# rust-cv/cv

Measured on NVIDIA H100. Metric: vSLAM frames/s (AKAZE+match+RANSAC, 1080p ~5k kp) at 1/2/4/8 H100, higher is better.
Workload: dtype f32+f64

## Files before the change

cv_b200/csrc/akaze.cu:

```cuda
#include <math.h>
#include <stdarg.h>
#include <stdio.h>
#include <stdlib.h>
#include <string.h>
#include <algorithm>
#include <atomic>
#include <vector>
#include "../../include/cvb200_stages.h"
#include "akaze_kernels.cuh"
#include "common.cuh"

using namespace akz;

namespace {

struct EvoHost {
    int w = 0, h = 0;
    uint32_t octave = 0, sublevel = 0;
    double esigma = 0, etime = 0;
    uint32_t sigma = 0;
    float quat = 0;
    float norm = 0, middle = 0;
    std::vector<double> tau;
    size_t off = 0;
// ... 104 lines not shown
    bool use_tma = false;
    int tma_mask = 3;
    SupScratch sup{};
    bool suppress_seq = false;
    bool suppress_par_only = false;
    unsigned *sup_fallback = nullptr;
    unsigned char *tile_evo = nullptr;
    MaskLayout mask_layout{};
    unsigned *extrema_mask = nullptr;
    bool deriv_v3 = true;
    OrientTables *ot = nullptr;
    DescTables *dt = nullptr;
    cvb_keypoint *kp_out = nullptr;
    unsigned char *desc_out = nullptr;
    unsigned *n_out = nullptr;
    unsigned cap_out = 0;
    std::vector<void *> allocs;
    std::vector<void *> kp_allocs;
    bool has_run = false;
    cudaStream_t aux = nullptr;
    cudaEvent_t ev_fork[8] = {}, ev_join = nullptr;
    struct GraphEntry { const void *img; void *kp, *desc, *n; unsigned B, cap; cudaGraphExec_t exec; };
    std::vector<GraphEntry> graphs;
    uint64_t launches_per_graph = 0;
    bool use_graph = true;
    bool use_aux = true;
    uint64_t ticket = 0;
    unsigned ss_batch = 0;
    DescTables *dt_side = nullptr;
    int dt_side_pattern = 0, dt_side_nch = 0;
    cvb_keypoint *st_kp = nullptr, *st_kp_out = nullptr;
    unsigned char *st_ok = nullptr, *st_desc = nullptr, *st_desc_out = nullptr;
    unsigned *st_off = nullptr, *st_n = nullptr, *st_need = nullptr;
    size_t st_kp_n = 0, st_kp_out_n = 0, st_ok_n = 0, st_desc_n = 0, st_desc_out_n = 0, st_off_n = 0, st_n_n = 0, st_need_n = 0;
};

void akaze_workspace_free(AkazeWorkspace *ws) {
    if (!ws) return;
    for (auto &g : ws->graphs) cudaGraphExecDestroy(g.exec);
    if (ws->aux) cudaStreamDestroy(ws->aux);
    for (cudaEvent_t e : ws->ev_fork) if (e) cudaEventDestroy(e);
    if (ws->ev_join) cudaEventDestroy(ws->ev_join);
    for (void *p : ws->allocs) cudaFree(p);
    for (void *p : ws->kp_allocs) cudaFree(p);
    for (void *p : {(void *)ws->st_kp, (void *)ws->st_kp_out, (void *)ws->st_ok, (void *)ws->st_desc, (void *)ws->st_desc_out,
                    (void *)ws->st_off, (void *)ws->st_n, (void *)ws->st_need})
        if (p) cudaFree(p);
    delete ws;
}

namespace {

#ifndef CVB_TMA_DEFAULT
#define CVB_TMA_DEFAULT 1
#endif
typedef CUresult (*EncodeTiledFn)(CUtensorMap *, CUtensorMapDataType, cuuint32_t, void *, const cuuint64_t *, const cuuint64_t *,
                                  const cuuint32_t *, const cuuint32_t *, CUtensorMapInterleave, CUtensorMapSwizzle, CUtensorMapL2promotion,
                                  CUtensorMapFloatOOBfill);
EncodeTiledFn encode_tiled_fn() {
    static EncodeTiledFn fn = nullptr;
    static bool tried = false;
    if (!tried) {
        tried = true;
        void *p = nullptr;
        cudaDriverEntryPointQueryResult qr;
        if (cudaGetDriverEntryPoint("cuTensorMapEncodeTiled", &p, cudaEnableDefault, &qr) == cudaSuccess && qr == cudaDriverEntryPointSuccess)
            fn = (EncodeTiledFn)p;
    }
    return fn;
}
bool make_tmap(CUtensorMap *out, const float *base, int w, int h, unsigned B, size_t bstride, int boxw, int boxh) {
    EncodeTiledFn fn = encode_tiled_fn();
    memset(out, 0, sizeof(*out));
    if (!fn || ((uintptr_t)base & 15) || (w & 3) || (bstride & 3) || boxw > 256 || boxh > 256 || w < 1 || h < 1) return false;
    const cuuint64_t dims[3] = {(cuuint64_t)w, (cuuint64_t)h, (cuuint64_t)std::max(B, 1u)};
    const cuuint64_t strides[2] = {(cuuint64_t)w * 4, (cuuint64_t)(B > 1 ? bstride : (size_t)w * h) * 4};
    const cuuint32_t box[3] = {(cuuint32_t)boxw, (cuuint32_t)boxh, 1};
    const cuuint32_t es[3] = {1, 1, 1};
    return fn(out, CU_TENSOR_MAP_DATA_TYPE_FLOAT32, 3, (void *)base, dims, strides, box, es, CU_TENSOR_MAP_INTERLEAVE_NONE,
              CU_TENSOR_MAP_SWIZZLE_NONE, CU_TENSOR_MAP_L2_PROMOTION_NONE, CU_TENSOR_MAP_FLOAT_OOB_FILL_NONE) == CUDA_SUCCESS;
}


int fed_fuse_steps() {
    static int v = 0;
    if (!v) { const char *env = getenv("CVB_FED_FUSE"); v = env ? std::min(std::max(atoi(env), 1), FED_SMAX) : FED_FUSE_DEFAULT; }
    return v;
}

template <typename T>
int dalloc_into(cvb_ctx *ctx, std::vector<void *> &list, T **p, size_t n) {
    void *q = nullptr;
    cudaError_t e = cudaMalloc(&q, std::max<size_t>(n, 1) * sizeof(T));
    if (e != cudaSuccess) return cvb_set_error(ctx, CVB_ENOMEM, "cudaMalloc(%zu bytes): %s", n * sizeof(T), cudaGetErrorString(e));
    list.push_back(q);
    *p = (T *)q;
    return 0;
}

template <typename T>
int dalloc(cvb_ctx *ctx, AkazeWorkspace *ws, T **p, size_t n) { return dalloc_into(ctx, ws->allocs, p, n); }

int alloc_keypoint_buffers(cvb_ctx *ctx, AkazeWorkspace *ws) {
    const size_t B = ws->batch;
    int rc = 0;
#define DK(p, n) do { rc = dalloc_into(ctx, ws->kp_allocs, &ws->p, (n)); if (rc) return rc; } while (0)
    DK(cand, B * ws->capc);
    DK(sup.state, B * ws->capc); DK(sup.alive, B * ws->capc); DK(sup.rdy, B * ws->capc);
    DK(sup.key, B * ws->capc); DK(sup.rank, B * ws->capc); DK(sup.next, B * ws->capc);
    DK(cache, B * ws->capk); DK(refined, B * ws->capk); DK(sorted, B * ws->capk); DK(rank, B * ws->capk);
    DK(keep, B * ws->capk); DK(valid, B * ws->capk); DK(ok, B * ws->capk); DK(desc_tmp, B * ws->capk * 64);
#undef DK
    return 0;
}

int grow_keypoint_capacity(cvb_ctx *ctx, AkazeWorkspace *ws, size_t need_c, size_t need_k) {
    CVB_CUDA(ctx, cvb_wait(ctx, ctx->stream));
    for (auto &g : ws->graphs) cudaGraphExecDestroy(g.exec);
    ws->graphs.clear();
    AkazeWorkspace *nw = new AkazeWorkspace();
    nw->batch = ws->batch;
    nw->capc = need_c > ws->capc ? (unsigned)std::min<size_t>(need_c + need_c / 8, 0xffffffffu) : ws->capc;
    nw->capk = need_k > ws->capk ? (unsigned)std::min<size_t>(need_k + need_k / 8, 0xffffffffu) : ws->capk;
    const int rc = alloc_keypoint_buffers(ctx, nw);
    if (rc) {
        for (void *p : nw->kp_allocs) cudaFree(p);
        delete nw;
        return rc;
    }
    for (void *p : ws->kp_allocs) cudaFree(p);
    ws->kp_allocs = std::move(nw->kp_allocs);
    ws->capc = nw->capc; ws->capk = nw->capk;
    ws->cand = nw->cand;
    ws->sup.state = nw->sup.state; ws->sup.alive = nw->sup.alive; ws->sup.rdy = nw->sup.rdy;
    ws->sup.key = nw->sup.key; ws->sup.rank = nw->sup.rank; ws->sup.next = nw->sup.next;
    ws->cache = nw->cache; ws->refined = nw->refined; ws->sorted = nw->sorted; ws->rank = nw->rank;
    ws->keep = nw->keep; ws->valid = nw->valid; ws->ok = nw->ok; ws->desc_tmp = nw->desc_tmp;
    delete nw;
    return 0;
}

bool same_cfg(const cvb_akaze_cfg &a, const cvb_akaze_cfg &b) { return memcmp(&a, &b, sizeof(a)) == 0; }

int plan_evolutions(cvb_ctx *ctx, AkazeWorkspace *ws) {
    const cvb_akaze_cfg &c = ws->cfg;
    ws->evo.clear();
    for (uint32_t octave = 0; octave < c.max_octave_evolution; octave++) {
        double rfactor = 1.0 / (double)(1ull << octave);
        uint32_t lh = (uint32_t)((double)ws->h * rfactor), lw = (uint32_t)((double)ws->w * rfactor);
        uint32_t smallest = std::min(lw, lh);
        if (smallest < 40) continue;
        uint32_t sub = smallest < 80 ? 1 : c.num_sublevels;
        for (uint32_t s = 0; s < sub; s++) {
            EvoHost e;
            e.octave = octave; e.sublevel = s;
            e.esigma = c.base_scale_offset * pow(2.0, (double)s / (double)c.num_sublevels + (double)octave);
            e.etime = 0.5 * (e.esigma * e.esigma);
            ws->evo.push_back(e);
        }
    }
    if (ws->evo.empty()) return 0;
    if (ws->evo.size() > (size_t)MAX_EVO) return cvb_set_error(ctx, CVB_EUNSUPPORTED, "more than %d evolutions", MAX_EVO);
    int lw = (int)ws->w, lh = (int)ws->h;
    size_t off = 0;
    int rowbase = 0, tilebase = 0;
    for (size_t i = 0; i < ws->evo.size(); i++) {
        EvoHost &e = ws->evo[i];
        e.new_octave = i > 0 && e.octave > ws->evo[i - 1].octave;
        if (e.new_octave) { lw /= 2; lh /= 2; }
        e.w = lw; e.h = lh; e.off = off;
        off += (size_t)lw * lh;
        off = (off + 63) & ~(size_t)63;
// ... 333 lines not shown
            dim3 g((unsigned)(t1 - t0), 1, B);
            CVB_PROF(ctx, "k_detector_response", 16.0 * px * B);
            k_detector_response<<<g, NT, sizeof(float) * det_smem_floats(smax), ds>>>(ws->Lsm, ws->Lt, ws->Lx, ws->Ly, ws->Ldet, PF, ws->table,
                                                                                      ws->tile_evo, t0, ws->mask_layout, thr, ws->extrema_mask,
                                                                                      ws->rowcount);
            CVB_LAUNCH_CHECK(ctx);
        } else if (ws->deriv_v3) {
            const size_t region = (((size_t)pitch3(smax) * (SH3 + 2 * smax)) + 31) & ~(size_t)31;
            dim3 g((unsigned)(t1 - t0), 1, B);
            { CVB_PROF(ctx, "k_deriv1", 12.0 * px * B);
            k_deriv1_v3<<<g, NT, sizeof(float) * region + 128, ds>>>(ws->Lsm, ws->Lt, ws->Lx, ws->Ly, PF, ws->table, ws->tile_evo, t0,
                                                               ws->use_tma && (ws->tma_mask & 4) ? ws->tmaps : nullptr);
            CVB_LAUNCH_CHECK(ctx); }
            { CVB_PROF(ctx, "k_deriv2_det", 12.0 * px * B);
            k_deriv2_v3<<<g, NT, sizeof(float) * 2 * region + 128, ds>>>(ws->Lx, ws->Ly, ws->Ldet, PF, ws->table, ws->tile_evo, t0,
                                                                   ws->use_tma && (ws->tma_mask & 8) ? ws->tmaps + MAX_EVO : nullptr, ws->use_tma && (ws->tma_mask & 8) ? ws->tmaps + 2 * MAX_EVO : nullptr);
            CVB_LAUNCH_CHECK(ctx); }
        } else {
            cudaStream_t keep = ctx->stream;
            ctx->stream = ds;
            int rc2 = 0;
            for (int e = e0; e < e1 && !rc2; e++) {
                const EvoHost &ev = ws->evo[e];
                rc2 = launch_deriv1(ctx, ev, (e == 0 ? ws->Lt : ws->Lsm) + ev.off, ws->Lx + ev.off, ws->Ly + ev.off, PF, B);
                if (!rc2) rc2 = launch_deriv2(ctx, ev, ws->Lx + ev.off, ws->Ly + ev.off, ws->Ldet + ev.off, PF, B);
            }
            ctx->stream = keep;
            if (rc2) return rc2;
        }
        return 0;
    };
    int octave_first = 0;
    int rc = launch_separable(ctx, images, P0, ws->Lt + ws->evo[0].off, PF, W, H, B, ws->g0, ws->g0);
    if (rc) return rc;
    CVB_CUDA(ctx, cudaMemsetAsync(ws->gmax, 0, sizeof(unsigned long long) * B, st));
    CVB_CUDA(ctx, cudaMemsetAsync(ws->hist, 0, sizeof(unsigned) * B * nbins, st));
    CVB_CUDA(ctx, cudaMemsetAsync(ws->npoints, 0, sizeof(unsigned) * B, st));
    CVB_CUDA(ctx, cudaMemsetAsync(ws->rowcount, 0, sizeof(unsigned) * (size_t)B * R, st));
    rc = launch_separable(ctx, images, P0, ws->tmpA, P0, W, H, B, ws->g1, ws->g1);
    if (rc) return rc;
    { CVB_PROF(ctx, "k_contrast_grad", 4.0 * W * H * B);
    k_scharr_pm_v3<1><<<dim3(cdiv((unsigned)W, SW3), cdiv((unsigned)H, SH3), B), NT, 0, st>>>(ws->tmpA, nullptr, ws->g2, ws->gmax, W, H, P0, P0, nullptr, 0);
    CVB_LAUNCH_CHECK(ctx); }
    {
        unsigned blocks = std::min<unsigned>(cdiv((unsigned)P0, NT), (unsigned)ctx->num_sms * 8);
        { CVB_PROF(ctx, "k_contrast_hist", 4.0 * W * H * B);
        k_contrast_hist<<<dim3(blocks, 1, B), NT, sizeof(unsigned) * nbins, st>>>(ws->g2, ws->gmax, ws->hist, ws->npoints, (int)P0, P0, nbins);
        CVB_LAUNCH_CHECK(ctx); }
        { CVB_PROF(ctx, "k_contrast_final", 0);
        k_contrast_final<<<B, 32, 0, st>>>(ws->gmax, ws->hist, ws->npoints, nbins, ws->cfg.contrast_percentile, ws->evo_octave, E, ws->kc, ws->inv_k);
        CVB_LAUNCH_CHECK(ctx); }
    }
    for (int i = 1; i < E; i++) {
        const EvoHost &e = ws->evo[i];
        const EvoHost &pe = ws->evo[i - 1];
        const float *src = ws->Lt + pe.off;
        size_t src_bs = PF;
        if (e.new_octave) {
            if ((rc = issue_detector_response(octave_first, i))) return rc;
            octave_first = i;
            dim3 blk(32, 8), grd(cdiv((unsigned)e.w, 32), cdiv((unsigned)e.h, 8), B);
            { CVB_PROF(ctx, "k_half_size", 4.0 * ((double)pe.w * pe.h + (double)e.w * e.h) * B);
            k_half_size<<<grd, blk, 0, st>>>(src, ws->tmpC, pe.w, pe.h, src_bs, P0);
            CVB_LAUNCH_CHECK(ctx); }
            src = ws->tmpC; src_bs = P0;
        }
        if (ws->fuse_blur_scharr && ws->g1.ks == 5) {
            CVB_PROF(ctx, "k_blur_scharr", 16.0 * e.w * e.h * B);
            CUtensorMap tm;
            const int use_tma = ws->use_tma && (ws->tma_mask & 2) && make_tmap(&tm, src, e.w, e.h, B, src_bs, pitch3(3), SH3 + 6) ? 1 : 0;
            if (!use_tma) memset(&tm, 0, sizeof(tm));
            k_blur_scharr_pm<<<dim3(cdiv((unsigned)e.w, SW3), cdiv((unsigned)e.h, SH3), B), NT, 0, st>>>(
                src, ws->Lsm + e.off, ws->Lflow + e.off, e.w, e.h, src_bs, PF, PF, ws->g1, ws->inv_k + i, MAX_EVO, tm, use_tma);
            CVB_LAUNCH_CHECK(ctx);
        } else {
            rc = launch_separable(ctx, src, src_bs, ws->Lsm + e.off, PF, e.w, e.h, B, ws->g1, ws->g1);
            if (rc) return rc;
            { CVB_PROF(ctx, "k_scharr_pm", 8.0 * e.w * e.h * B);
            k_scharr_pm_v3<0><<<dim3(cdiv((unsigned)e.w, SW3), cdiv((unsigned)e.h, SH3), B), NT, 0, st>>>(ws->Lsm + e.off, ws->Lflow + e.off, nullptr, nullptr, e.w, e.h, PF, PF,
                                                                 ws->inv_k + i, MAX_EVO);
            CVB_LAUNCH_CHECK(ctx); }
        }
        const int n = (int)e.tau.size();
        const int fed_fuse = fed_fuse_steps();
        const int nl = (n + fed_fuse - 1) / fed_fuse;
        if (nl == 0) {
            CVB_CUDA(ctx, cudaMemcpy2DAsync(ws->Lt + e.off, PF * sizeof(float), src, src_bs * sizeof(float),
                                            (size_t)e.w * e.h * sizeof(float), B, cudaMemcpyDeviceToDevice, st));
        }
        const float *cur = src; size_t cur_bs = src_bs;
        int done = 0;
        for (int l = 0; l < nl; l++) {
            FedSteps fs;
            fs.n = (n - done + (nl - l) - 1) / (nl - l);
            for (int t = 0; t < fs.n; t++) fs.tau[t] = (float)e.tau[(size_t)(done + t)];
            done += fs.n;
            float *dst; size_t dst_bs;
            if (l == nl - 1) { dst = ws->Lt + e.off; dst_bs = PF; }
            else if (((nl - 1 - l) & 1) == 1) { dst = ws->tmpA; dst_bs = P0; }
            else { dst = ws->tmpB; dst_bs = P0; }
            { CVB_PROF(ctx, "k_fed", 12.0 * fs.n * e.w * e.h * B);
            const int hx = (fs.n + 3) & ~3;
            dim3 grd(cdiv((unsigned)e.w, (unsigned)(F3_W - 2 * hx)), cdiv((unsigned)e.h, (unsigned)(F3_H - 2 * fs.n)), B);
            k_fed3<<<grd, F3_H * 16, 0, st>>>(cur, ws->Lflow + e.off, dst, e.w, e.h, cur_bs, PF, dst_bs, fs);
            CVB_LAUNCH_CHECK(ctx); }
            cur = dst; cur_bs = dst_bs;
        }
    }
    if ((rc = issue_detector_response(octave_first, E))) return rc;
    if (forked) {
        CVB_CUDA(ctx, cudaEventRecord(ws->ev_join, ws->aux));
        CVB_CUDA(ctx, cudaStreamWaitEvent(st, ws->ev_join, 0));
    }
    return 0;
}

int stage_detect(cvb_ctx *ctx, unsigned B) {
    AkazeWorkspace *ws = ctx->akaze;
    cudaStream_t st = ctx->stream;
    const size_t PF = ws->plane_floats;
    const bool fused_det = ws->deriv_v3 && ws->fuse_det;
    const int R = ws->table.total_rows;
    const float thr = (float)ws->cfg.detector_threshold;
    {
        if (!fused_det) { CVB_PROF(ctx, "k_extrema_mask", 4.0 * ws->plane_floats * B);
        k_extrema_mask<<<dim3((unsigned)ws->table.total_tiles, 1, B), NT, 0, st>>>(ws->Ldet, PF, ws->table, ws->tile_evo, ws->mask_layout, thr,
                                                                                    ws->extrema_mask, ws->rowcount);
        CVB_LAUNCH_CHECK(ctx); }
        { CVB_PROF(ctx, "k_scan_rows", 0);
        k_scan_rows<<<B, 1024, 0, st>>>(ws->rowcount, ws->rowoff, ws->ncand, R);
        CVB_LAUNCH_CHECK(ctx); }
        { CVB_PROF(ctx, "k_extrema_emit", 0);
        k_extrema_emit<<<dim3(cdiv((unsigned)R * 32u, NT), 1, B), NT, 0, st>>>(ws->Ldet, PF, ws->table, ws->mask_layout, ws->extrema_mask, ws->rowcount,
                                                                                 ws->rowoff, ws->cand, ws->capc, ws->overflow);
        CVB_LAUNCH_CHECK(ctx); }
    }
    { CVB_PROF(ctx, "k_suppress", 0);
    if (ws->suppress_seq)
        k_suppress_seq<<<B, 1024, 0, st>>>(ws->cand, ws->ncand, ws->capc, ws->table, ws->cache, ws->ncache, ws->nneed, ws->capk,
                                           ws->overflow);
    else {
        k_suppress_smem<<<B, 1024, SUP_SMEM, st>>>(ws->cand, ws->ncand, ws->rowoff, ws->capc, ws->table, ws->sup, ws->cache,
                                                   ws->ncache, ws->nneed, ws->capk, ws->overflow, ws->sup_fallback);
        CVB_LAUNCH_CHECK(ctx);
        k_suppress_par<<<B, 1024, 0, st>>>(ws->cand, ws->ncand, ws->rowoff, ws->capc, ws->table, ws->sup, ws->cache, ws->ncache,
                                           ws->nneed, ws->capk, ws->overflow, ws->suppress_par_only ? nullptr : ws->sup_fallback);
    }
    CVB_LAUNCH_CHECK(ctx); }
    const unsigned kp_blocks = (unsigned)ctx->num_sms * 2;
    const unsigned ichunks = std::min<unsigned>(cdiv(ws->capk, NT), 64u);
    CVB_CUDA(ctx, cudaMemsetAsync(ws->keep, 1, (size_t)B * ws->capk, st));
    { CVB_PROF(ctx, "k_filter_upper", 0);
    k_filter_upper<<<dim3(ichunks, 16, B), NT, 0, st>>>(ws->cache, ws->ncache, ws->capk, ws->keep);
    CVB_LAUNCH_CHECK(ctx); }
    { CVB_PROF(ctx, "k_refine_orient", 0);
    k_refine_orient<<<dim3(kp_blocks, B), NT, 0, st>>>(ws->cache, ws->ncache, ws->capk, ws->keep, ws->table, ws->Ldet, ws->Lx, ws->Ly, PF,
                                                       ws->ot, ws->refined, ws->valid);
    CVB_LAUNCH_CHECK(ctx); }
    return 0;
}

int stage_sort_describe(cvb_ctx *ctx, unsigned B, cvb_keypoint *kp_out, unsigned char *desc_out, unsigned cap_out, unsigned *n_out) {
    AkazeWorkspace *ws = ctx->akaze;
    cudaStream_t st = ctx->stream;
    const size_t PF = ws->plane_floats;
    const unsigned ichunks = std::min<unsigned>(cdiv(ws->capk, NT), 64u);
    CVB_CUDA(ctx, cudaMemsetAsync(ws->rank, 0, sizeof(unsigned) * (size_t)B * ws->capk, st));
    CVB_CUDA(ctx, cudaMemsetAsync(ws->nvalid, 0, sizeof(unsigned) * B, st));
    { CVB_PROF(ctx, "k_rank_sort", 0);
    k_rank_count<<<dim3(ichunks, 16, B), NT, 0, st>>>(ws->refined, ws->valid, ws->ncache, ws->capk, ws->rank);
    CVB_LAUNCH_CHECK(ctx);
    k_rank_scatter<<<dim3(ichunks, B), NT, 0, st>>>(ws->refined, ws->valid, ws->ncache, ws->capk, ws->rank,
                                                    (long long)ws->cfg.maximum_features, ws->sorted, ws->nvalid);
    CVB_LAUNCH_CHECK(ctx);
    k_clamp_count<<<cdiv(B, 32), 32, 0, st>>>(ws->nvalid, (long long)ws->cfg.maximum_features, ws->nsorted, (int)B);
    CVB_LAUNCH_CHECK(ctx); }
    { CVB_PROF(ctx, "k_descriptors", 0);
    k_descriptors<<<dim3((unsigned)ctx->num_sms * 8, B), DESC_WARPS * 32, 0, st>>>(ws->sorted, ws->nsorted, nullptr, ws->capk, ws->table, ws->Lt,
                                                     ws->Lx, ws->Ly, PF, ws->dt, (int)ws->cfg.descriptor_channels,
                                                     (int)ws->cfg.descriptor_pattern_size, ws->desc_tmp, ws->ok, ws->overflow);
    CVB_LAUNCH_CHECK(ctx); }
    { CVB_PROF(ctx, "k_compact_final", 0);
    k_compact_final<<<B, 1024, 0, st>>>(ws->sorted, ws->desc_tmp, ws->ok, ws->nsorted, ws->capk, kp_out, desc_out, cap_out, n_out,
                                        ws->overflow);
    CVB_LAUNCH_CHECK(ctx); }
    return 0;
}
// ... 486 lines not shown
```

cv_b200/csrc/akaze_kernels.cuh:

```cuda
#pragma once
#include <cuda.h>
#include <cuda/barrier>
#include <cuda_runtime.h>
#include <stdint.h>
#include "device_libm.cuh"
#include "../../include/cvb200.h"

namespace akz {

constexpr int TW = 32;
constexpr int TH = 32;
constexpr int NT = 256;
constexpr int MAXK = 33;
constexpr int MAX_EVO = 32;
constexpr int MAX_TAU = 64;
constexpr int FED_SMAX = 8, FED_FUSE_DEFAULT = 8;

struct Taps { int ks; float k[MAXK]; };

struct EvoDev {
    int w, h;
    unsigned long long off;
    int octave;
    float size;
    int rowbase;
    int tilebase;
    int sigma;
    float norm, middle;
    float quat;
    int pad;
};
struct EvoTable { int n; int total_rows; int total_tiles; int pad; EvoDev e[MAX_EVO]; };

struct Cand { int x, y, e; float v; };

__device__ __forceinline__ int clampi(int v, int lo, int hi) { return v < lo ? lo : (v > hi ? hi : v); }

__device__ __forceinline__ float lane_dot(const float *w, int stride, const float *k, int ks) {
    float l0 = 0.f, l1 = 0.f, l2 = 0.f, l3 = 0.f;
    int j = 0;
    for (; j + 4 <= ks; j += 4) {
        l0 = w[(j + 0) * stride] * k[j + 0] + l0;
        l1 = w[(j + 1) * stride] * k[j + 1] + l1;
        l2 = w[(j + 2) * stride] * k[j + 2] + l2;
        l3 = w[(j + 3) * stride] * k[j + 3] + l3;
    }
    if (j < ks) l0 = w[j * stride] * k[j] + l0;
    if (j + 1 < ks) l1 = w[(j + 1) * stride] * k[j + 1] + l1;
    if (j + 2 < ks) l2 = w[(j + 2) * stride] * k[j + 2] + l2;
    return (l0 + l2) + (l1 + l3);
}

template <int JA, int JB>
__device__ __forceinline__ float dot2(float a, float ka, float b, float kb) {
    return (a * ka + b * kb) + 0.f;
}
template <int JA, int JB, int JC>
__device__ __forceinline__ float dot3(float a, float ka, float b, float kb, float c, float kc) {
    const float pa = a * ka, pb = b * kb, pc = c * kc;
    float r;
    if (JA == JB) r = (JC == JA) ? pc + (pb + pa) : (pb + pa) + pc;
    else if (JA == JC) r = (pc + pa) + pb;
    else if (JB == JC) r = (pc + pb) + pa;
    else if ((JA ^ JB) == 2) r = (pa + pb) + pc;
    else if ((JA ^ JC) == 2) r = (pa + pc) + pb;
    else r = (pb + pc) + pa;
    return r + 0.f;
}
template <int SM>
__device__ __forceinline__ float scharr_main(float first, float last) {
    return (last - first) + 0.f;
}
template <int SM>
__device__ __forceinline__ float scharr_off(float first, float mid, float last, float norm, float middle) {
    return dot3<0, SM & 3, (2 * SM) & 3>(first, norm, mid, middle, last, norm);
}

__global__ void __launch_bounds__(NT) k_separable(const float *__restrict__ in, float *__restrict__ out, int w, int h,
                                                  size_t in_bstride, size_t out_bstride, Taps hk, Taps vk) {
    extern __shared__ float sm[];
    const int rx = hk.ks / 2, ry = vk.ks / 2;
    const int sw = TW + 2 * rx, sh = TH + 2 * ry;
    float *s_in = sm;
    float *s_h = sm + sh * sw;
    const float *src = in + (size_t)blockIdx.z * in_bstride;
    float *dst = out + (size_t)blockIdx.z * out_bstride;
    const int x0 = blockIdx.x * TW, y0 = blockIdx.y * TH;
    for (int i = threadIdx.x; i < sw * sh; i += NT) {
        int ly = i / sw, lx = i - ly * sw;
        int gx = clampi(x0 + lx - rx, 0, w - 1), gy = clampi(y0 + ly - ry, 0, h - 1);
        s_in[i] = src[(size_t)gy * w + gx];
    }
    __syncthreads();
    for (int i = threadIdx.x; i < TW * sh; i += NT) {
        int ly = i / TW, lx = i - ly * TW;
        s_h[i] = lane_dot(s_in + ly * sw + lx, 1, hk.k, hk.ks);
    }
    __syncthreads();
    for (int i = threadIdx.x; i < TW * TH; i += NT) {
        int ly = i / TW, lx = i - ly * TW;
        int gx = x0 + lx, gy = y0 + ly;
        if (gx < w && gy < h) dst[(size_t)gy * w + gx] = lane_dot(s_h + ly * TW + lx, TW, vk.k, vk.ks);
    }
}

__global__ void k_half_size(const float *__restrict__ in, float *__restrict__ out, int w, int h, size_t in_bstride,
                            size_t out_bstride) {
    const int hw = w / 2, hh = h / 2;
    const int x = blockIdx.x * blockDim.x + threadIdx.x, y = blockIdx.y * blockDim.y + threadIdx.y;
    if (x >= hw || y >= hh) return;
    const float *p = in + (size_t)blockIdx.z * in_bstride;
    const bool oddw = hw * 2 != w, oddh = hh * 2 != h;
    float v;
    if (oddw && oddh && x == hw - 1 && y == hh - 1) v = p[(size_t)(h - 1) * w + (w - 1)];
    else if (oddw && x == hw - 1) v = (p[(size_t)(2 * y) * w + (w - 1)] + p[(size_t)(2 * y + 1) * w + (w - 1)]) * 0.5f;
    else if (oddh && y == hh - 1) v = (p[(size_t)(h - 1) * w + 2 * x] + p[(size_t)(h - 1) * w + 2 * x + 1]) * 0.5f;
    else {
        const float *q = p + (size_t)(2 * y) * w + 2 * x;
        v = ((q[0] + q[1]) + (q[w] + q[w + 1])) * 0.25f;
    }
    out[(size_t)blockIdx.z * out_bstride + (size_t)y * hw + x] = v;
}

__global__ void __launch_bounds__(NT) k_contrast_hist(const double *__restrict__ g2, const unsigned long long *gmax,
                                                      unsigned *hist, unsigned *npoints, int n, size_t bstride, int nbins) {
    extern __shared__ unsigned s_hist[];
    for (int i = threadIdx.x; i < nbins; i += NT) s_hist[i] = 0;
    __syncthreads();
    const double hmax = sqrt(__longlong_as_double((long long)gmax[blockIdx.z]));
    const double *p = g2 + (size_t)blockIdx.z * bstride;
    unsigned cnt = 0;
    for (int i = blockIdx.x * NT + threadIdx.x; i < n; i += gridDim.x * NT) {
        double v = p[i];
        if (v < 0.0) continue;
        double modg = sqrt(v);
        if (modg != 0.0) {
            long long bin = (long long)floor((double)nbins * (modg / hmax));
            if (bin == nbins) bin -= 1;
            if (bin >= 0 && bin < nbins) atomicAdd(&s_hist[bin], 1u);
            cnt++;
        }
    }
    __syncthreads();
    for (int i = threadIdx.x; i < nbins; i += NT)
        if (s_hist[i]) atomicAdd(&hist[(size_t)blockIdx.z * nbins + i], s_hist[i]);
    for (int o = 16; o; o >>= 1) cnt += __shfl_down_sync(0xffffffffu, cnt, o);
    if ((threadIdx.x & 31) == 0 && cnt) atomicAdd(&npoints[blockIdx.z], cnt);
}

__global__ void k_contrast_final(const unsigned long long *gmax, const unsigned *hist, const unsigned *npoints, int nbins,
                                 double percentile, const int *evo_octave, int nevo, double *kc, float *inv_k) {
    const int b = blockIdx.x;
    if (threadIdx.x != 0) return;
    const double hmax = sqrt(__longlong_as_double((long long)gmax[b]));
    const double num_points = (double)npoints[b];
    const unsigned long long threshold = (unsigned long long)(num_points * percentile);
    unsigned long long k = 0, nel = 0;
    while (nel < threshold && k < (unsigned long long)nbins) { nel += hist[(size_t)b * nbins + k]; k++; }
    double c = (nel >= threshold) ? hmax * (double)k / (double)nbins : 0.03;
    kc[b] = c;
    for (int i = 1; i < nevo; i++) {
        if (evo_octave[i] > evo_octave[i - 1]) c *= 0.75;
        inv_k[(size_t)b * MAX_EVO + i] = (float)(1.0 / (c * c));
    }
}

struct FedSteps { int n; float tau[FED_SMAX]; };

constexpr int F3_W = 128, F3_H = 32;
template <bool BORDER>
__device__ __forceinline__ void fed3_steps(float (&l)[2][4], const float (&cH)[2][5], const float (&cV)[3][4], float *cur,
                                           float *nxt, const float *s_hs, int S, int lx0, int ly0, int gx0, int gy0,
                                           int w, int h) {
    const int rowU = max(ly0 - 1, 0) * F3_W + lx0, rowD = min(ly0 + 2, F3_H - 1) * F3_W + lx0, row0 = ly0 * F3_W + lx0;
    for (int t = 0; t < S; t++) {
        const float hs = s_hs[t];
        float lL[2], lR[2];
#pragma unroll
        for (int r = 0; r < 2; r++) {
            lL[r] = __shfl_up_sync(0xffffffffu, l[r][3], 1);
            lR[r] = __shfl_down_sync(0xffffffffu, l[r][0], 1);
        }
        const float4 up4 = *reinterpret_cast<const float4 *>(cur + rowU), dn4 = *reinterpret_cast<const float4 *>(cur + rowD);
        const float up[4] = {up4.x, up4.y, up4.z, up4.w}, dn[4] = {dn4.x, dn4.y, dn4.z, dn4.w};
        float fh[2][5], fv[3][4];
#pragma unroll
        for (int r = 0; r < 2; r++) {
            fh[r][0] = (hs * cH[r][0]) * (l[r][0] - lL[r]);
#pragma unroll
            for (int e = 1; e < 4; e++) fh[r][e] = (hs * cH[r][e]) * (l[r][e] - l[r][e - 1]);
            fh[r][4] = (hs * cH[r][4]) * (lR[r] - l[r][3]);
        }
#pragma unroll
        for (int k = 0; k < 4; k++) {
            fv[0][k] = (hs * cV[0][k]) * (l[0][k] - up[k]);
            fv[1][k] = (hs * cV[1][k]) * (l[1][k] - l[0][k]);
            fv[2][k] = (hs * cV[2][k]) * (dn[k] - l[1][k]);
        }
#pragma unroll
        for (int r = 0; r < 2; r++)
#pragma unroll
            for (int k = 0; k < 4; k++) {
                float v = l[r][k];
                if (BORDER) {
                    const int gx = gx0 + k, gy = gy0 + r;
                    v = gx < w - 1 ? v + fh[r][k + 1] : v;
                    v = gx > 0 ? v - fh[r][k] : v;
                    v = gy < h - 1 ? v + fv[r + 1][k] : v;
                    v = gy > 0 ? v - fv[r][k] : v;
                } else {
                    v = v + fh[r][k + 1];
                    v = v - fh[r][k];
                    v = v + fv[r + 1][k];
                    v = v - fv[r][k];
                }
                l[r][k] = v;
            }
        if (t + 1 < S) {
            *reinterpret_cast<float4 *>(nxt + row0) = make_float4(l[0][0], l[0][1], l[0][2], l[0][3]);
            *reinterpret_cast<float4 *>(nxt + row0 + F3_W) = make_float4(l[1][0], l[1][1], l[1][2], l[1][3]);
            __syncthreads();
            float *tmp = cur; cur = nxt; nxt = tmp;
        }
    }
}

__global__ void __launch_bounds__(F3_H * 16, 2) k_fed3(const float *__restrict__ Lin, const float *__restrict__ C,
                                                       float *__restrict__ Lout, int w, int h, size_t lin_bstride,
                                                       size_t c_bstride, size_t lout_bstride, FedSteps steps) {
    __shared__ __align__(16) float bufA[F3_H * F3_W], bufB[F3_H * F3_W];
    __shared__ float s_hs[FED_SMAX];
    const int S = steps.n, HX = (S + 3) & ~3;
    if (threadIdx.x < FED_SMAX) s_hs[threadIdx.x] = 0.5f * steps.tau[threadIdx.x];
    const int tw = F3_W - 2 * HX, th = F3_H - 2 * S;
    const int lx0 = (threadIdx.x & 31) * 4, ly0 = (threadIdx.x >> 5) * 2;
    const int X0 = blockIdx.x * tw - HX, Y0 = blockIdx.y * th - S;
    const int gx0 = X0 + lx0, gy0 = Y0 + ly0;
    const float *lin = Lin + (size_t)blockIdx.z * lin_bstride;
    const float *cc = C + (size_t)blockIdx.z * c_bstride;
    const bool vec = (w & 3) == 0;
    float l[2][4], c[2][4];
#pragma unroll
    for (int r = 0; r < 2; r++) {
        const int gy = gy0 + r;
        const bool rowin = gy >= 0 && gy < h;
        const size_t g = (size_t)gy * w + gx0;
        if (vec) {
            float4 a = make_float4(0.f, 0.f, 0.f, 0.f), b = a;
            if (rowin && gx0 >= 0 && gx0 < w) { a = *reinterpret_cast<const float4 *>(lin + g); b = *reinterpret_cast<const float4 *>(cc + g); }
            l[r][0] = a.x; l[r][1] = a.y; l[r][2] = a.z; l[r][3] = a.w;
            c[r][0] = b.x; c[r][1] = b.y; c[r][2] = b.z; c[r][3] = b.w;
        } else {
#pragma unroll
            for (int k = 0; k < 4; k++) {
                const bool in = rowin && gx0 + k >= 0 && gx0 + k < w;
                l[r][k] = in ? lin[g + k] : 0.f;
                c[r][k] = in ? cc[g + k] : 0.f;
            }
        }
        *reinterpret_cast<float4 *>(bufA + (ly0 + r) * F3_W + lx0) = make_float4(l[r][0], l[r][1], l[r][2], l[r][3]);
        *reinterpret_cast<float4 *>(bufB + (ly0 + r) * F3_W + lx0) = make_float4(c[r][0], c[r][1], c[r][2], c[r][3]);
    }
    __syncthreads();
    float cH[2][5], cV[3][4];
    {
#pragma unroll
        for (int r = 0; r < 2; r++) {
            const float cl = __shfl_up_sync(0xffffffffu, c[r][3], 1), cr = __shfl_down_sync(0xffffffffu, c[r][0], 1);
            cH[r][0] = cl + c[r][0];
#pragma unroll
            for (int e = 1; e < 4; e++) cH[r][e] = c[r][e - 1] + c[r][e];
            cH[r][4] = c[r][3] + cr;
        }
        const float4 cu4 = *reinterpret_cast<const float4 *>(bufB + max(ly0 - 1, 0) * F3_W + lx0);
        const float4 cd4 = *reinterpret_cast<const float4 *>(bufB + min(ly0 + 2, F3_H - 1) * F3_W + lx0);
        const float cu[4] = {cu4.x, cu4.y, cu4.z, cu4.w}, cd[4] = {cd4.x, cd4.y, cd4.z, cd4.w};
#pragma unroll
        for (int k = 0; k < 4; k++) { cV[0][k] = cu[k] + c[0][k]; cV[1][k] = c[0][k] + c[1][k]; cV[2][k] = c[1][k] + cd[k]; }
    }
    __syncthreads();
    const bool border = X0 <= 0 || Y0 <= 0 || X0 + F3_W >= w || Y0 + F3_H >= h;
    if (border) fed3_steps<true>(l, cH, cV, bufA, bufB, s_hs, S, lx0, ly0, gx0, gy0, w, h);
    else fed3_steps<false>(l, cH, cV, bufA, bufB, s_hs, S, lx0, ly0, gx0, gy0, w, h);
    float *dst = Lout + (size_t)blockIdx.z * lout_bstride;
    if (lx0 >= HX && lx0 < F3_W - HX && gx0 < w) {
#pragma unroll
        for (int r = 0; r < 2; r++) {
            const int ly = ly0 + r, gy = gy0 + r;
            if (ly < S || ly >= F3_H - S || gy >= h) continue;
            const size_t g = (size_t)gy * w + gx0;
            if (vec) *reinterpret_cast<float4 *>(dst + g) = make_float4(l[r][0], l[r][1], l[r][2], l[r][3]);
            else {
#pragma unroll
                for (int k = 0; k < 4; k++) if (gx0 + k < w) dst[g + k] = l[r][k];
            }
        }
    }
}

template <int SM>
__global__ void __launch_bounds__(NT) k_deriv1(const float *__restrict__ Ls, float *__restrict__ Lx,
                                               float *__restrict__ Ly, int w, int h, size_t bstride, int sigma,
                                               float norm, float middle) {
    extern __shared__ float sm[];
    const int sw = TW + 2 * sigma, sh = TH + 2 * sigma;
    float *s_in = sm;
    float *s_hm = sm + sh * sw;
    float *s_ho = s_hm + sh * TW;
    const float *src = Ls + (size_t)blockIdx.z * bstride;
    const int x0 = blockIdx.x * TW, y0 = blockIdx.y * TH;
    for (int i = threadIdx.x; i < sw * sh; i += NT) {
        int ly = i / sw, lx = i - ly * sw;
        int gx = clampi(x0 + lx - sigma, 0, w - 1), gy = clampi(y0 + ly - sigma, 0, h - 1);
        s_in[i] = src[(size_t)gy * w + gx];
    }
    __syncthreads();
    for (int i = threadIdx.x; i < TW * sh; i += NT) {
        int ly = i / TW, lx = i - ly * TW;
        const float *p = s_in + ly * sw + lx;
        s_hm[i] = scharr_main<SM>(p[0], p[2 * sigma]);
        s_ho[i] = scharr_off<SM>(p[0], p[sigma], p[2 * sigma], norm, middle);
    }
    __syncthreads();
    for (int i = threadIdx.x; i < TW * TH; i += NT) {
        int ly = i / TW, lx = i - ly * TW;
        int gx = x0 + lx, gy = y0 + ly;
        if (gx >= w || gy >= h) continue;
        const float *pm = s_hm + ly * TW + lx, *po = s_ho + ly * TW + lx;
        size_t g = (size_t)blockIdx.z * bstride + (size_t)gy * w + gx;
        Lx[g] = scharr_off<SM>(pm[0], pm[sigma * TW], pm[2 * sigma * TW], norm, middle);
        Ly[g] = scharr_main<SM>(po[0], po[2 * sigma * TW]);
    }
}

template <int SM>
__global__ void __launch_bounds__(NT) k_deriv2_det(const float *__restrict__ Lx, const float *__restrict__ Ly,
                                                   float *__restrict__ Ldet, int w, int h, size_t bstride, int sigma,
                                                   float norm, float middle, float quat) {
    extern __shared__ float sm[];
    const int sw = TW + 2 * sigma, sh = TH + 2 * sigma;
    float *s_x = sm;
    float *s_y = sm + sh * sw;
    float *s_a = s_y + sh * sw;
    float *s_b = s_a + sh * TW;
    float *s_c = s_b + sh * TW;
    const float *px = Lx + (size_t)blockIdx.z * bstride, *py = Ly + (size_t)blockIdx.z * bstride;
    const int x0 = blockIdx.x * TW, y0 = blockIdx.y * TH;
    for (int i = threadIdx.x; i < sw * sh; i += NT) {
        int ly = i / sw, lx = i - ly * sw;
        int gx = clampi(x0 + lx - sigma, 0, w - 1), gy = clampi(y0 + ly - sigma, 0, h - 1);
        size_t g = (size_t)gy * w + gx;
        s_x[i] = px[g];
        s_y[i] = py[g];
    }
    __syncthreads();
    for (int i = threadIdx.x; i < TW * sh; i += NT) {
        int ly = i / TW, lx = i - ly * TW;
        const float *p = s_x + ly * sw + lx, *q = s_y + ly * sw + lx;
        s_a[i] = scharr_main<SM>(p[0], p[2 * sigma]);
        s_b[i] = scharr_off<SM>(q[0], q[sigma], q[2 * sigma], norm, middle);
        s_c[i] = scharr_off<SM>(p[0], p[sigma], p[2 * sigma], norm, middle);
    }
    __syncthreads();
    for (int i = threadIdx.x; i < TW * TH; i += NT) {
        int ly = i / TW, lx = i - ly * TW;
        int gx = x0 + lx, gy = y0 + ly;
        if (gx >= w || gy >= h) continue;
        const float *pa = s_a + ly * TW + lx, *pb = s_b + ly * TW + lx, *pc = s_c + ly * TW + lx;
        float lxx = scharr_off<SM>(pa[0], pa[sigma * TW], pa[2 * sigma * TW], norm, middle);
        float lyy = scharr_main<SM>(pb[0], pb[2 * sigma * TW]);
        float lxy = scharr_main<SM>(pc[0], pc[2 * sigma * TW]);
        Ldet[(size_t)blockIdx.z * bstride + (size_t)gy * w + gx] = (lxx * lyy - lxy * lxy) * quat;
// ... 1494 lines not shown
```

Baseline: 1593.

## Restructure fused FED kernel to 3 rows per warp with edge-only shared exchange

Rewrites the fused FED diffusion kernel so each warp owns three rows (48-row tile, 16 warps) instead of two rows in a 32-row tile. Only the top and bottom rows of each warp go through double-buffered shared memory each step, and the interior vertical neighbours stay in registers. Conductivity sums are computed on the fly rather than precomputed. The maximum number of fused steps rises from 8 to 12, which cuts launch count and relative halo overhead, and the CVB_FED_FUSE environment knob is removed. In exchange the kernel carries more register pressure and uses a larger FedSteps parameter block.

```diff
diff --git a/cv_b200/csrc/akaze.cu b/cv_b200/csrc/akaze.cu
--- a/cv_b200/csrc/akaze.cu
+++ b/cv_b200/csrc/akaze.cu
@@ -210,12 +210,6 @@
 }
 
 
-int fed_fuse_steps() {
-    static int v = 0;
-    if (!v) { const char *env = getenv("CVB_FED_FUSE"); v = env ? std::min(std::max(atoi(env), 1), FED_SMAX) : FED_FUSE_DEFAULT; }
-    return v;
-}
-
 template <typename T>
 int dalloc_into(cvb_ctx *ctx, std::vector<void *> &list, T **p, size_t n) {
     void *q = nullptr;
@@ -715,8 +709,7 @@
             CVB_LAUNCH_CHECK(ctx); }
         }
         const int n = (int)e.tau.size();
-        const int fed_fuse = fed_fuse_steps();
-        const int nl = (n + fed_fuse - 1) / fed_fuse;
+        const int nl = (n + FED_SMAX - 1) / FED_SMAX;
         if (nl == 0) {
             CVB_CUDA(ctx, cudaMemcpy2DAsync(ws->Lt + e.off, PF * sizeof(float), src, src_bs * sizeof(float),
                                             (size_t)e.w * e.h * sizeof(float), B, cudaMemcpyDeviceToDevice, st));
@@ -733,9 +726,8 @@
             else if (((nl - 1 - l) & 1) == 1) { dst = ws->tmpA; dst_bs = P0; }
             else { dst = ws->tmpB; dst_bs = P0; }
             { CVB_PROF(ctx, "k_fed", 12.0 * fs.n * e.w * e.h * B);
-            const int hx = (fs.n + 3) & ~3;
-            dim3 grd(cdiv((unsigned)e.w, (unsigned)(F3_W - 2 * hx)), cdiv((unsigned)e.h, (unsigned)(F3_H - 2 * fs.n)), B);
-            k_fed3<<<grd, F3_H * 16, 0, st>>>(cur, ws->Lflow + e.off, dst, e.w, e.h, cur_bs, PF, dst_bs, fs);
+            dim3 grd(cdiv((unsigned)e.w, (unsigned)(FED_W - 2 * fed_hx(fs.n))), cdiv((unsigned)e.h, (unsigned)(FED_H - 2 * fs.n)), B);
+            k_fed<<<grd, FED_NW * 32, 0, st>>>(cur, ws->Lflow + e.off, dst, e.w, e.h, cur_bs, PF, dst_bs, fs);
             CVB_LAUNCH_CHECK(ctx); }
             cur = dst; cur_bs = dst_bs;
         }
diff --git a/cv_b200/csrc/akaze_kernels.cuh b/cv_b200/csrc/akaze_kernels.cuh
--- a/cv_b200/csrc/akaze_kernels.cuh
+++ b/cv_b200/csrc/akaze_kernels.cuh
@@ -14,7 +14,6 @@
 constexpr int MAXK = 33;
 constexpr int MAX_EVO = 32;
 constexpr int MAX_TAU = 64;
-constexpr int FED_SMAX = 8, FED_FUSE_DEFAULT = 8;
 
 struct Taps { int ks; float k[MAXK]; };
 
@@ -165,83 +164,76 @@
     }
 }
 
-struct FedSteps { int n; float tau[FED_SMAX]; };
-
-constexpr int F3_W = 128, F3_H = 32;
+struct FedSteps { int n; float tau[MAX_TAU]; };
+
+constexpr int FED_W = 128, FED_RH = 3, FED_NW = 16, FED_H = FED_RH * FED_NW;
+constexpr int FED_SMAX = 12;
+__host__ __device__ constexpr int fed_hx(int s) { return (s + 3) & ~3; }
 template <bool BORDER>
-__device__ __forceinline__ void fed3_steps(float (&l)[2][4], const float (&cH)[2][5], const float (&cV)[3][4], float *cur,
-                                           float *nxt, const float *s_hs, int S, int lx0, int ly0, int gx0, int gy0,
-                                           int w, int h) {
-    const int rowU = max(ly0 - 1, 0) * F3_W + lx0, rowD = min(ly0 + 2, F3_H - 1) * F3_W + lx0, row0 = ly0 * F3_W + lx0;
+__device__ __forceinline__ void fed_steps(float (&l)[FED_RH][4], const float (&c)[FED_RH][4], const float (&cL)[FED_RH],
+                                          const float (&cR)[FED_RH], const float (&cU)[4], const float (&cD)[4], float *s_edge, const float *s_hs, int S, int warp, int lx0, int gx0, int gy0, int w, int h) {
+    const int up = max(warp - 1, 0) * FED_W + lx0, dn = min(warp + 1, FED_NW - 1) * FED_W + lx0, own = warp * FED_W + lx0;
     for (int t = 0; t < S; t++) {
+        float *top = s_edge + (t & 1) * 2 * FED_NW * FED_W, *bot = top + FED_NW * FED_W;
+        *reinterpret_cast<float4 *>(top + own) = make_float4(l[0][0], l[0][1], l[0][2], l[0][3]);
+        *reinterpret_cast<float4 *>(bot + own) = make_float4(l[FED_RH - 1][0], l[FED_RH - 1][1], l[FED_RH - 1][2], l[FED_RH - 1][3]);
+        __syncthreads();
         const float hs = s_hs[t];
-        float lL[2], lR[2];
-#pragma unroll
-        for (int r = 0; r < 2; r++) {
-            lL[r] = __shfl_up_sync(0xffffffffu, l[r][3], 1);
-            lR[r] = __shfl_down_sync(0xffffffffu, l[r][0], 1);
-        }
-        const float4 up4 = *reinterpret_cast<const float4 *>(cur + rowU), dn4 = *reinterpret_cast<const float4 *>(cur + rowD);
-        const float up[4] = {up4.x, up4.y, up4.z, up4.w}, dn[4] = {dn4.x, dn4.y, dn4.z, dn4.w};
-        float fh[2][5], fv[3][4];
-#pragma unroll
-        for (int r = 0; r < 2; r++) {
-            fh[r][0] = (hs * cH[r][0]) * (l[r][0] - lL[r]);
-#pragma unroll
-            for (int e = 1; e < 4; e++) fh[r][e] = (hs * cH[r][e]) * (l[r][e] - l[r][e - 1]);
-            fh[r][4] = (hs * cH[r][4]) * (lR[r] - l[r][3]);
-        }
-#pragma unroll
-        for (int k = 0; k < 4; k++) {
-            fv[0][k] = (hs * cV[0][k]) * (l[0][k] - up[k]);
-            fv[1][k] = (hs * cV[1][k]) * (l[1][k] - l[0][k]);
-            fv[2][k] = (hs * cV[2][k]) * (dn[k] - l[1][k]);
-        }
-#pragma unroll
-        for (int r = 0; r < 2; r++)
+        const float4 u4 = *reinterpret_cast<const float4 *>(bot + up), d4 = *reinterpret_cast<const float4 *>(top + dn);
+        const float lu[4] = {u4.x, u4.y, u4.z, u4.w}, ld[4] = {d4.x, d4.y, d4.z, d4.w};
+        float fu[4];
+#pragma unroll
+        for (int k = 0; k < 4; k++) fu[k] = (hs * cU[k]) * (l[0][k] - lu[k]);
+#pragma unroll
+        for (int r = 0; r < FED_RH; r++) {
+            const float lL = __shfl_up_sync(0xffffffffu, l[r][3], 1), lR = __shfl_down_sync(0xffffffffu, l[r][0], 1);
+            float fh[5], fd[4];
+            fh[0] = (hs * cL[r]) * (l[r][0] - lL);
+#pragma unroll
+            for (int e = 1; e < 4; e++) fh[e] = (hs * (c[r][e - 1] + c[r][e])) * (l[r][e] - l[r][e - 1]);
+            fh[4] = (hs * cR[r]) * (lR - l[r][3]);
+#pragma unroll
+            for (int k = 0; k < 4; k++)
+                fd[k] = (hs * (r + 1 < FED_RH ? c[r][k] + c[r + 1][k] : cD[k])) * ((r + 1 < FED_RH ? l[r + 1][k] : ld[k]) - l[r][k]);
 #pragma unroll
             for (int k = 0; k < 4; k++) {
                 float v = l[r][k];
                 if (BORDER) {
                     const int gx = gx0 + k, gy = gy0 + r;
-                    v = gx < w - 1 ? v + fh[r][k + 1] : v;
-                    v = gx > 0 ? v - fh[r][k] : v;
-                    v = gy < h - 1 ? v + fv[r + 1][k] : v;
-                    v = gy > 0 ? v - fv[r][k] : v;
+                    v = gx < w - 1 ? v + fh[k + 1] : v;
+                    v = gx > 0 ? v - fh[k] : v;
+                    v = gy < h - 1 ? v + fd[k] : v;
+                    v = gy > 0 ? v - fu[k] : v;
                 } else {
-                    v = v + fh[r][k + 1];
-                    v = v - fh[r][k];
-                    v = v + fv[r + 1][k];
-                    v = v - fv[r][k];
+                    v = v + fh[k + 1];
+                    v = v - fh[k];
+                    v = v + fd[k];
+                    v = v - fu[k];
                 }
                 l[r][k] = v;
-            }
-        if (t + 1 < S) {
-            *reinterpret_cast<float4 *>(nxt + row0) = make_float4(l[0][0], l[0][1], l[0][2], l[0][3]);
-            *reinterpret_cast<float4 *>(nxt + row0 + F3_W) = make_float4(l[1][0], l[1][1], l[1][2], l[1][3]);
-            __syncthreads();
-            float *tmp = cur; cur = nxt; nxt = tmp;
-        }
-    }
-}
-
-__global__ void __launch_bounds__(F3_H * 16, 2) k_fed3(const float *__restrict__ Lin, const float *__restrict__ C,
-                                                       float *__restrict__ Lout, int w, int h, size_t lin_bstride,
-                                                       size_t c_bstride, size_t lout_bstride, FedSteps steps) {
-    __shared__ __align__(16) float bufA[F3_H * F3_W], bufB[F3_H * F3_W];
-    __shared__ float s_hs[FED_SMAX];
-    const int S = steps.n, HX = (S + 3) & ~3;
-    if (threadIdx.x < FED_SMAX) s_hs[threadIdx.x] = 0.5f * steps.tau[threadIdx.x];
-    const int tw = F3_W - 2 * HX, th = F3_H - 2 * S;
-    const int lx0 = (threadIdx.x & 31) * 4, ly0 = (threadIdx.x >> 5) * 2;
+                fu[k] = fd[k];
+            }
+        }
+    }
+}
+
+__global__ void __launch_bounds__(FED_NW * 32, 2) k_fed(const float *__restrict__ Lin, const float *__restrict__ C,
+                                                        float *__restrict__ Lout, int w, int h, size_t lin_bstride,
+                                                        size_t c_bstride, size_t lout_bstride, FedSteps steps) {
+    __shared__ __align__(16) float s_edge[2 * 2 * FED_NW * FED_W];
+    __shared__ float s_hs[MAX_TAU];
+    const int S = steps.n, HX = fed_hx(S);
+    if (threadIdx.x < S) s_hs[threadIdx.x] = 0.5f * steps.tau[threadIdx.x];
+    const int tw = FED_W - 2 * HX, th = FED_H - 2 * S;
+    const int warp = threadIdx.x >> 5, lx0 = (threadIdx.x & 31) * 4, ly0 = warp * FED_RH;
     const int X0 = blockIdx.x * tw - HX, Y0 = blockIdx.y * th - S;
     const int gx0 = X0 + lx0, gy0 = Y0 + ly0;
     const float *lin = Lin + (size_t)blockIdx.z * lin_bstride;
     const float *cc = C + (size_t)blockIdx.z * c_bstride;
     const bool vec = (w & 3) == 0;
-    float l[2][4], c[2][4];
-#pragma unroll
-    for (int r = 0; r < 2; r++) {
+    float l[FED_RH][4], c[FED_RH][4];
+#pragma unroll
+    for (int r = 0; r < FED_RH; r++) {
         const int gy = gy0 + r;
         const bool rowin = gy >= 0 && gy < h;
         const size_t g = (size_t)gy * w + gx0;
@@ -258,36 +250,34 @@
                 c[r][k] = in ? cc[g + k] : 0.f;
             }
         }
-        *reinterpret_cast<float4 *>(bufA + (ly0 + r) * F3_W + lx0) = make_float4(l[r][0], l[r][1], l[r][2], l[r][3]);
-        *reinterpret_cast<float4 *>(bufB + (ly0 + r) * F3_W + lx0) = make_float4(c[r][0], c[r][1], c[r][2], c[r][3]);
-    }
-    __syncthreads();
-    float cH[2][5], cV[3][4];
+    }
+    float cL[FED_RH], cR[FED_RH], cU[4], cD[4];
     {
-#pragma unroll
-        for (int r = 0; r < 2; r++) {
+        float *top = s_edge + 2 * FED_NW * FED_W, *bot = top + FED_NW * FED_W;
+        *reinterpret_cast<float4 *>(top + warp * FED_W + lx0) = make_float4(c[0][0], c[0][1], c[0][2], c[0][3]);
+        *reinterpret_cast<float4 *>(bot + warp * FED_W + lx0) = make_float4(c[FED_RH - 1][0], c[FED_RH - 1][1], c[FED_RH - 1][2], c[FED_RH - 1][3]);
+#pragma unroll
+        for (int r = 0; r < FED_RH; r++) {
             const float cl = __shfl_up_sync(0xffffffffu, c[r][3], 1), cr = __shfl_down_sync(0xffffffffu, c[r][0], 1);
-            cH[r][0] = cl + c[r][0];
-#pragma unroll
-            for (int e = 1; e < 4; e++) cH[r][e] = c[r][e - 1] + c[r][e];
-            cH[r][4] = c[r][3] + cr;
-        }
-        const float4 cu4 = *reinterpret_cast<const float4 *>(bufB + max(ly0 - 1, 0) * F3_W + lx0);
-        const float4 cd4 = *reinterpret_cast<const float4 *>(bufB + min(ly0 + 2, F3_H - 1) * F3_W + lx0);
+            cL[r] = cl + c[r][0];
+            cR[r] = c[r][3] + cr;
+        }
+        __syncthreads();
+        const float4 cu4 = *reinterpret_cast<const float4 *>(bot + max(warp - 1, 0) * FED_W + lx0);
+        const float4 cd4 = *reinterpret_cast<const float4 *>(top + min(warp + 1, FED_NW - 1) * FED_W + lx0);
         const float cu[4] = {cu4.x, cu4.y, cu4.z, cu4.w}, cd[4] = {cd4.x, cd4.y, cd4.z, cd4.w};
 #pragma unroll
-        for (int k = 0; k < 4; k++) { cV[0][k] = cu[k] + c[0][k]; cV[1][k] = c[0][k] + c[1][k]; cV[2][k] = c[1][k] + cd[k]; }
-    }
-    __syncthreads();
-    const bool border = X0 <= 0 || Y0 <= 0 || X0 + F3_W >= w || Y0 + F3_H >= h;
-    if (border) fed3_steps<true>(l, cH, cV, bufA, bufB, s_hs, S, lx0, ly0, gx0, gy0, w, h);
-    else fed3_steps<false>(l, cH, cV, bufA, bufB, s_hs, S, lx0, ly0, gx0, gy0, w, h);
+        for (int k = 0; k < 4; k++) { cU[k] = cu[k] + c[0][k]; cD[k] = c[FED_RH - 1][k] + cd[k]; }
+    }
+    const bool border = X0 <= 0 || Y0 <= 0 || X0 + FED_W >= w || Y0 + FED_H >= h;
+    if (border) fed_steps<true>(l, c, cL, cR, cU, cD, s_edge, s_hs, S, warp, lx0, gx0, gy0, w, h);
+    else fed_steps<false>(l, c, cL, cR, cU, cD, s_edge, s_hs, S, warp, lx0, gx0, gy0, w, h);
     float *dst = Lout + (size_t)blockIdx.z * lout_bstride;
-    if (lx0 >= HX && lx0 < F3_W - HX && gx0 < w) {
-#pragma unroll
-        for (int r = 0; r < 2; r++) {
+    if (lx0 >= HX && lx0 < FED_W - HX && gx0 < w) {
+#pragma unroll
+        for (int r = 0; r < FED_RH; r++) {
             const int ly = ly0 + r, gy = gy0 + r;
-            if (ly < S || ly >= F3_H - S || gy >= h) continue;
+            if (ly < S || ly >= FED_H - S || gy >= h) continue;
             const size_t g = (size_t)gy * w + gx0;
             if (vec) *reinterpret_cast<float4 *>(dst + g) = make_float4(l[r][0], l[r][1], l[r][2], l[r][3]);
             else {
```

Result: faster. 1623, median of 6 (+1.9%).
